# pearl-robot-lab/2HandedAfforder

Measured on AMD Instinct MI355X. Metric: affordance frames/sec/GPU @1024^2, 32-tok prompt; mask IoU vs ref, higher is better.
Workload: dtype bf16

## Files before the change

2handedafforder_amd/csrc/window_attention.hip:

```cpp
#include "haff_common.h"

#ifndef HAFF_TUNING
#undef HAFF_WIN_NOKREAD
#undef HAFF_WIN_NOVREAD
#undef HAFF_WIN_NOSCR
#undef HAFF_WIN_NODMA
#undef HAFF_WIN_RS
#undef HAFF_WIN_KLAST_OLD
#endif

namespace {

struct WinArgs {
  const bf16_t *q, *k, *v;
  bf16_t* o;
  long q_sb, q_sh, q_st;
  long k_sb, k_sh, k_st;
  long v_sb, v_sh, v_st;
  long o_sb, o_sh, o_st;
  int B, H;
  float scale;
  const bf16_t *tab_h, *tab_w;
  int grid_h, grid_w, wps;
  long pad_token;
};

#ifdef HAFF_WIN_TRACE
__device__ unsigned long long haff_win_trace_buf[64 * 16];
#define WTRACE(i) do { if (blockIdx.x == 0 && tid == 0 && it < 64) haff_win_trace_buf[it * 16 + (i)] = wall_clock64(); } while (0)
#else
#define WTRACE(i) do {} while (0)
#endif

constexpr float WLOG2E = 1.4426950408889634f;
typedef __attribute__((address_space(3))) bf16x4* wlds_v4_ptr;
typedef const __attribute__((address_space(1))) void* wgptr_t;
typedef __attribute__((address_space(3))) void* wlptr_t;
__device__ __attribute__((aligned(16))) unsigned int haff_win_zero_page[4];

template <int D, int S>
struct WinCfg {
  static constexpr int N = S * S;
  static constexpr int NKD = (D + 31) / 32;
  static constexpr int ND = D / 16;
  static constexpr int CPR = D / 8;
  static constexpr int KPC = (D * 2) % 64 == 32 ? 0 : 2;
  static constexpr int KSTR = D * 2 + 16 * KPC;
  static constexpr int VSTR = D * 2;
  static constexpr int NKS = (S + 1) / 2;
#ifdef HAFF_WIN_RS
  static constexpr int RS = HAFF_WIN_RS;
#else
  static constexpr int RS = 52;
#endif
  static constexpr int QPW = 2;
  static constexpr int NWAVES = (S + QPW - 1) / QPW;
  static constexpr int NTHREADS = 64 * NWAVES;
  static constexpr int KSLOTS = N * (CPR + KPC), VSLOTS = N * CPR;
  static constexpr int K_BYTES = N * KSTR, V_BYTES = N * VSTR;
  static constexpr int PAD_SLOTS = (KSLOTS + VSLOTS + 63) / 64 * 64;
  static constexpr int BUF_BYTES = PAD_SLOTS * 16;
  static constexpr int SC_BYTES = NWAVES * 16 * RS * 4;
  static constexpr int LDS_BYTES = 2 * BUF_BYTES + SC_BYTES;
};

template <int D, int S, bool F16 = false>
__global__ __launch_bounds__((WinCfg<D, S>::NTHREADS)) void window_attn_kernel(WinArgs p) {
  using E = h16<F16>;
  using C = WinCfg<D, S>;
  static_assert(D % 16 == 0 && D <= 96 && S <= 16 && 2 * S - 1 <= 32, "window kernel geometry");
  extern __shared__ __attribute__((aligned(16))) unsigned char wsm[];
  float* sScr = reinterpret_cast<float*>(wsm + 2 * C::BUF_BYTES);

  const int tid = threadIdx.x;
  const int lane = tid & 63;
  const int wave = __builtin_amdgcn_readfirstlane(tid >> 6);
  const int fr = lane & 15, fh = lane >> 4;
  const int n_items = p.B * p.H;

  auto decode = [&](int id, int& win, int& h) {
    if ((p.B & 7) == 0) {
      const int x = id & 7, kseq = id >> 3;
      win = (kseq / p.H) * 8 + x;
      h = kseq - (kseq / p.H) * p.H;
    } else {
      win = id / p.H;
      h = id - win * p.H;
    }
  };

  constexpr int TOTAL_SLOTS = C::KSLOTS + C::VSLOTS;
  constexpr int NDMA = (C::PAD_SLOTS + C::NTHREADS - 1) / C::NTHREADS;
  static_assert((C::K_BYTES % 16) == 0 && C::KSTR == (C::CPR + C::KPC) * 16 && C::VSTR == C::CPR * 16 && C::KSTR % 64 == 32, "slot layout");
  unsigned slot_off[NDMA];
  unsigned slot_pad[NDMA];
  const long v_minus_k = (p.v - p.k);
  const unsigned vmk_bytes = (unsigned)(v_minus_k * 2);
#pragma unroll
  for (int i = 0; i < NDMA; ++i) {
    const int sl = tid + i * C::NTHREADS;
    long off;
    unsigned pad = 0;
    if (sl >= TOTAL_SLOTS) {
      off = 0;
    } else if (sl < C::KSLOTS) {
      const int row = sl / (C::CPR + C::KPC), c = sl - row * (C::CPR + C::KPC);
      off = (long)row * p.k_st + (c < C::CPR ? c * 8 : 0);
      pad = ((unsigned)(row / S) << 28) | ((unsigned)(row % S) << 24) | (unsigned)((c < C::CPR ? c : 0) * 16);
    } else {
      const int sv = sl - C::KSLOTS;
      const int row = sv / C::CPR, c = sv - row * C::CPR;
      off = v_minus_k + (long)row * p.v_st + c * 8;
      pad = ((unsigned)(row / S) << 28) | ((unsigned)(row % S) << 24) | (1u << 23) | (unsigned)(c * 16);
    }
    slot_off[i] = (unsigned)(off * 2);
    slot_pad[i] = pad;
  }
  uint4 qnext[C::QPW][C::NKD];
  const int qcol = min(fr, S - 1);
  const bf16_t* nx_kb = p.k;
  int nx_pad_h0 = S, nx_pad_w0 = S;
  unsigned nx_pad_base = 0, nx_lds0 = 0;
  auto begin_loads = [&](int id, int buf) {
    int win, h;
    decode(id, win, h);
    const bf16_t* qb = p.q + (long)win * p.q_sb + (long)h * p.q_sh;
    const bf16_t* kb = p.k + (long)win * p.k_sb + (long)h * p.k_sh;
    int pad_h0 = S, pad_w0 = S;
    if (p.grid_h > 0) {
      const int wi = win % (p.wps * p.wps);
      pad_h0 = p.grid_h - (wi / p.wps) * S;
      pad_w0 = p.grid_w - (wi % p.wps) * S;
    }
    const unsigned pad_base = (unsigned)((p.pad_token * p.k_st - (long)win * p.k_sb) * 2);
    const bf16_t* qpad = p.q + p.pad_token * p.q_st + (long)h * p.q_sh;
#pragma unroll
    for (int t = 0; t < C::QPW; ++t) {
      const int qh_t = min(wave + t * C::NWAVES, S - 1);
      const bf16_t* qsrc = (qh_t >= pad_h0 || qcol >= pad_w0) ? qpad : qb + (long)(qh_t * S + qcol) * p.q_st;
#pragma unroll
      for (int kd = 0; kd < C::NKD; ++kd) {
        const int col = kd * 32 + fh * 8;
        qnext[t][kd] = make_uint4(0, 0, 0, 0);
        if (col < D) qnext[t][kd] = *reinterpret_cast<const uint4*>(qsrc + col);
      }
    }
    nx_kb = kb;
    nx_pad_h0 = pad_h0;
    nx_pad_w0 = pad_w0;
    nx_pad_base = pad_base;
    nx_lds0 = (unsigned)(uintptr_t)(wlptr_t)(wsm + buf * C::BUF_BYTES) + wave * 1024;
  };
  auto issue_dma = [&](int i0, int i1) {
#pragma unroll
    for (int i = 0; i < NDMA; ++i) {
      if (i < i0 || i >= i1) continue;
      const unsigned m0v = nx_lds0 + i * C::NTHREADS * 16;
      const bool is_pad = (int)(slot_pad[i] >> 28) >= nx_pad_h0 || (int)((slot_pad[i] >> 24) & 15u) >= nx_pad_w0;
      const unsigned off = is_pad ? nx_pad_base + (slot_pad[i] & 0xffu) + ((slot_pad[i] >> 23) & 1u) * vmk_bytes : slot_off[i];
#ifdef HAFF_WIN_NODMA
      asm volatile("" ::"v"(off), "s"(m0v));
      continue;
#endif
      if ((i + 1) * C::NTHREADS <= C::PAD_SLOTS || (i * C::NTHREADS + wave * 64) < C::PAD_SLOTS)
        asm volatile("s_mov_b32 m0, %2\n\ts_nop 0\n\tglobal_load_lds_dwordx4 %0, %1" ::"v"(off), "s"(nx_kb), "s"(m0v)
                     : "memory");
    }
  };
  constexpr int DMA_Q1 = (NDMA + 3) / 4, DMA_Q2 = (NDMA + 1) / 2, DMA_Q3 = (3 * NDMA + 3) / 4;

  auto settle_q = [&]() {
#pragma unroll
    for (int t = 0; t < C::QPW; ++t)
#pragma unroll
      for (int kd = 0; kd < C::NKD; ++kd)
        asm volatile("" : "+v"(qnext[t][kd].x), "+v"(qnext[t][kd].y), "+v"(qnext[t][kd].z), "+v"(qnext[t][kd].w));
  };

  int item = blockIdx.x;
  if (item >= n_items) return;
  begin_loads(item, 0);
  issue_dma(0, NDMA);

  bf16x8 th[2][C::NKD], tw[2][C::NKD];
#pragma unroll
  for (int mt = 0; mt < 2; ++mt) {
    const int r = min(mt * 16 + fr, 2 * S - 2);
#pragma unroll
    for (int kd = 0; kd < C::NKD; ++kd) {
      const int col = kd * 32 + fh * 8;
      uint4 a = make_uint4(0, 0, 0, 0), b = make_uint4(0, 0, 0, 0);
      if (col < D) {
        a = *reinterpret_cast<const uint4*>(p.tab_h + r * D + col);
        b = *reinterpret_cast<const uint4*>(p.tab_w + r * D + col);
      }
      th[mt][kd] = __builtin_bit_cast(bf16x8, a);
      tw[mt][kd] = __builtin_bit_cast(bf16x8, b);
    }
  }
  asm volatile("s_waitcnt vmcnt(0)" ::: "memory");
  settle_q();
#pragma unroll
  for (int mt = 0; mt < 2; ++mt)
#pragma unroll
    for (int kd = 0; kd < C::NKD; ++kd) {
      asm volatile("" : "+v"(th[mt][kd]));
      asm volatile("" : "+v"(tw[mt][kd]));
    }
  __syncthreads();

  const float sl2 = p.scale * WLOG2E;
  float* scr = sScr + wave * (16 * C::RS);
  const int tr_q = fr >> 2, tr_p = fr & 3;
  bool kw_ok[4];
#pragma unroll
  for (int j = 0; j < 4; ++j) kw_ok[j] = (4 * fh + j) < S;

  for (int it = 0;; ++it) {
    const int buf = it & 1;
    const unsigned char* sK = wsm + buf * C::BUF_BYTES;
    const unsigned char* sV = sK + C::K_BYTES;
    int win, h;
    decode(item, win, h);
    bf16_t* ob = p.o + (long)win * p.o_sb + (long)h * p.o_sh;
    uint4 qcur[C::QPW][C::NKD];
#pragma unroll
    for (int t = 0; t < C::QPW; ++t)
#pragma unroll
      for (int kd = 0; kd < C::NKD; ++kd) qcur[t][kd] = qnext[t][kd];
    const int next = item + gridDim.x;
    const bool has_next = next < n_items;
    WTRACE(0);
    if (has_next) {
      begin_loads(next, buf ^ 1);
      issue_dma(0, DMA_Q1);
    }
    WTRACE(1);

#pragma unroll
    for (int t = 0; t < C::QPW; ++t) {
      const int qh = wave + t * C::NWAVES;
      static_assert(C::QPW * C::NWAVES == S, "q-tiles must divide evenly over the waves");
      bf16x8 qraw[C::NKD], qs[C::NKD];
#pragma unroll
      for (int kd = 0; kd < C::NKD; ++kd) {
        const uint4 r = qcur[t][kd];
        uint4 rs = make_uint4(0, 0, 0, 0);
        if (kd * 32 + fh * 8 < D) {
          float qv[8];
          const unsigned w4[4] = {r.x, r.y, r.z, r.w};
#pragma unroll
          for (int j = 0; j < 4; ++j) {
            qv[2 * j] = E::lo(w4[j]) * sl2;
            qv[2 * j + 1] = E::hi(w4[j]) * sl2;
          }
          rs.x = E::pack2(qv[0], qv[1]); rs.y = E::pack2(qv[2], qv[3]);
          rs.z = E::pack2(qv[4], qv[5]); rs.w = E::pack2(qv[6], qv[7]);
        }
        qraw[kd] = __builtin_bit_cast(bf16x8, r);
        qs[kd] = __builtin_bit_cast(bf16x8, rs);
      }

      float relw4[4], relh_t[S];
      {
        f32x4 t0 = f32x4{0.f, 0.f, 0.f, 0.f}, t1 = t0;
#pragma unroll
        for (int kd = 0; kd < C::NKD; ++kd) {
          t0 = E::mfma16(tw[0][kd], qraw[kd], t0);
          t1 = E::mfma16(tw[1][kd], qraw[kd], t1);
        }
        float a[4] = {t0[0], t0[1], t0[2], t0[3]}, b[4] = {t1[0], t1[1], t1[2], t1[3]};
#ifdef HAFF_WIN_NOSCR
#pragma unroll
        for (int j = 0; j < 4; ++j) relw4[j] = kw_ok[j] ? (a[j] + b[j]) * WLOG2E : -INFINITY;
#else
        store4(scr + fr * C::RS + 4 * fh, a);
        store4(scr + fr * C::RS + 16 + 4 * fh, b);
        __builtin_amdgcn_wave_barrier();
#pragma unroll
        for (int j = 0; j < 4; ++j) {
          const int r = min(max(qcol - (4 * fh + j) + S - 1, 0), 2 * S - 2);
          relw4[j] = kw_ok[j] ? scr[fr * C::RS + r] * WLOG2E : -INFINITY;
        }
        __builtin_amdgcn_wave_barrier();
#endif
      }
      {
        f32x4 t0 = f32x4{0.f, 0.f, 0.f, 0.f}, t1 = t0;
#pragma unroll
        for (int kd = 0; kd < C::NKD; ++kd) {
          t0 = E::mfma16(th[0][kd], qraw[kd], t0);
          t1 = E::mfma16(th[1][kd], qraw[kd], t1);
        }
        float a[4] = {t0[0], t0[1], t0[2], t0[3]}, b[4] = {t1[0], t1[1], t1[2], t1[3]};
#ifdef HAFF_WIN_NOSCR
#pragma unroll
        for (int kt = 0; kt < S; ++kt) relh_t[kt] = (a[kt & 3] + b[kt & 3]) * WLOG2E;
#else
        store4(scr + fr * C::RS + 4 * fh, a);
        store4(scr + fr * C::RS + 16 + 4 * fh, b);
        __builtin_amdgcn_wave_barrier();
#pragma unroll
        for (int kt = 0; kt < S; ++kt) relh_t[kt] = scr[fr * C::RS + (qh - kt + S - 1)] * WLOG2E;
        __builtin_amdgcn_wave_barrier();
#endif
      }

      WTRACE(2 + 5 * t);
      f32x4 sacc[S];
#pragma unroll
      for (int kt = 0; kt < S; ++kt)
        sacc[kt] = f32x4{relw4[0] + relh_t[kt], relw4[1] + relh_t[kt], relw4[2] + relh_t[kt], relw4[3] + relh_t[kt]};
      constexpr int KG = (S + 1) / 2;
#ifdef HAFF_WIN_KLAST_OLD
      const int koff_last = min(fh * 16 + (C::NKD - 1) * 64, D * 2 - 16);
#else
      const int koff_last = (D * 2 - (C::NKD - 1) * 64 == 32) ? (C::NKD - 1) * 64 - 32 + ((fh + 2) & 3) * 16
                                                              : min(fh * 16 + (C::NKD - 1) * 64, D * 2 - 16);
#endif
#pragma unroll
      for (int g0 = 0; g0 < S; g0 += KG) {
#pragma unroll
        for (int kd = 0; kd < C::NKD; ++kd) {
#pragma unroll
          for (int kt = g0; kt < g0 + KG && kt < S; ++kt) {
#ifdef HAFF_WIN_NOKREAD
            const bf16x8 kf = qs[(kd + 1) % C::NKD];
#else
            const bf16x8 kf = *reinterpret_cast<const bf16x8*>(sK + (kt * S + qcol) * C::KSTR + (kd == C::NKD - 1 ? koff_last : fh * 16 + kd * 64));
#endif
            sacc[kt] = E::mfma16(kf, qs[kd], sacc[kt]);
          }
        }
        __builtin_amdgcn_sched_barrier(0);
      }

      WTRACE(3 + 5 * t);
      if (has_next) {
        if (t == 0) issue_dma(DMA_Q1, DMA_Q2);
        else issue_dma(DMA_Q3, NDMA);
      }
      float mx = -1e30f;
#pragma unroll
      for (int kt = 0; kt < S; ++kt)
#pragma unroll
        for (int j = 0; j < 4; ++j) mx = fmaxf(mx, sacc[kt][j]);
      mx = fmaxf(mx, __shfl_xor(mx, 16, 64));
      mx = fmaxf(mx, __shfl_xor(mx, 32, 64));
      float psum = 0.f;
#pragma unroll
      for (int kt = 0; kt < S; ++kt)
#pragma unroll
        for (int j = 0; j < 4; ++j) {
          const float e = __builtin_amdgcn_exp2f(sacc[kt][j] - mx);
          sacc[kt][j] = e;
          psum += e;
        }
      psum += __shfl_xor(psum, 16, 64);
      psum += __shfl_xor(psum, 32, 64);

      WTRACE(4 + 5 * t);
      f32x4 oacc[C::ND];
#pragma unroll
      for (int dt = 0; dt < C::ND; ++dt) oacc[dt] = f32x4{0.f, 0.f, 0.f, 0.f};
      const int vkw = min(4 * fh + tr_q, S - 1);
#pragma unroll
      for (int ks = 0; ks < C::NKS; ++ks) {
        constexpr int dummy = 0; (void)dummy;
        const int t0 = 2 * ks, t1 = (2 * ks + 1 < S) ? 2 * ks + 1 : 2 * ks;
        uint4 u;
        u.x = E::pack2(sacc[t0][0], sacc[t0][1]);
        u.y = E::pack2(sacc[t0][2], sacc[t0][3]);
        u.z = (2 * ks + 1 < S) ? E::pack2(sacc[t1][0], sacc[t1][1]) : 0u;
        u.w = (2 * ks + 1 < S) ? E::pack2(sacc[t1][2], sacc[t1][3]) : 0u;
        const bf16x8 pf = __builtin_bit_cast(bf16x8, u);
        const unsigned char* v0 = sV + (t0 * S + vkw) * C::VSTR + 8 * tr_p;
        const unsigned char* v1 = sV + (t1 * S + vkw) * C::VSTR + 8 * tr_p;
#pragma unroll
        for (int dt = 0; dt < C::ND; ++dt) {
#ifdef HAFF_WIN_NOVREAD
          const bf16x8 vf = qs[dt % C::NKD];
          asm volatile("" ::"v"(v0), "v"(v1));
#else
          const bf16x4 lo = __builtin_amdgcn_ds_read_tr16_b64_v4i16((wlds_v4_ptr)(v0 + 32 * dt));
          const bf16x4 hi = __builtin_amdgcn_ds_read_tr16_b64_v4i16((wlds_v4_ptr)(v1 + 32 * dt));
          const bf16x8 vf = __builtin_shufflevector(lo, hi, 0, 1, 2, 3, 4, 5, 6, 7);
#endif
          oacc[dt] = E::mfma16(vf, pf, oacc[dt]);
        }
      }

      WTRACE(5 + 5 * t);
      if (has_next && t == 0) issue_dma(DMA_Q2, DMA_Q3);
      const float inv = 1.0f / psum;
      if (fr < S) {
        bf16_t* orow = ob + (long)(qh * S + fr) * p.o_st + 4 * fh;
#pragma unroll
        for (int dt = 0; dt < C::ND; ++dt) {
          float v[4] = {oacc[dt][0] * inv, oacc[dt][1] * inv, oacc[dt][2] * inv, oacc[dt][3] * inv};
          store4h<F16>(orow + 16 * dt, v);
        }
      }
    }

    WTRACE(12);
    if (!has_next) break;
    item = next;
    asm volatile("s_waitcnt vmcnt(0)" ::: "memory");
    settle_q();
    WTRACE(13);
    __syncthreads();
    WTRACE(14);
  }
}

}

#ifdef HAFF_WIN_TRACE
extern "C" int haff_win_trace_read(unsigned long long* host, int n_words) {
  return hipMemcpyFromSymbol(host, HIP_SYMBOL(haff_win_trace_buf), sizeof(unsigned long long) * n_words) == hipSuccess ? 0 : 1;
}
#endif

template <bool F16 = false>
static int window_attention_impl(const void* q, long q_sb, long q_sh, long q_st,
                                 const void* k, long k_sb, long k_sh, long k_st,
                                 const void* v, long v_sb, long v_sh, long v_st,
                                 void* o, long o_sb, long o_sh, long o_st,
                                 int n_windows, int H, int S, int d, float scale,
                                 const void* tab_h, const void* tab_w, int grid_h, int grid_w,
                                 long pad_token, void* stream) {
  if (n_windows <= 0 || H <= 0 || S <= 0 || d <= 0 || !tab_h || !tab_w) return HAFF_ERR_BAD_ARG;
  if ((q_st & 7) || (k_st & 7) || (v_st & 7) || (o_st & 3) || (q_sh & 7) || (k_sh & 7) || (v_sh & 7) || (o_sh & 3) ||
      (q_sb & 7) || (k_sb & 7) || (v_sb & 7) || (o_sb & 3))
    return HAFF_ERR_BAD_ARG;
  if ((reinterpret_cast<uintptr_t>(q) & 15) || (reinterpret_cast<uintptr_t>(k) & 15) ||
      (reinterpret_cast<uintptr_t>(v) & 15) || (reinterpret_cast<uintptr_t>(o) & 7) ||
      (reinterpret_cast<uintptr_t>(tab_h) & 15) || (reinterpret_cast<uintptr_t>(tab_w) & 15))
    return HAFF_ERR_BAD_ARG;
  if (S != 14 || d != 80) return HAFF_ERR_UNSUPPORTED;
  if (k_sb != v_sb || k_sh != v_sh || k_st != v_st) return HAFF_ERR_UNSUPPORTED;
  {
    const long dvk = reinterpret_cast<const bf16_t*>(v) - reinterpret_cast<const bf16_t*>(k);
    const long span = (dvk < 0 ? -dvk : dvk) + (long)S * S * k_st + d;
    if (dvk < 0 || span * 2 >= (1L << 32)) return HAFF_ERR_UNSUPPORTED;
  }
  WinArgs p{reinterpret_cast<const bf16_t*>(q), reinterpret_cast<const bf16_t*>(k), reinterpret_cast<const bf16_t*>(v),
            reinterpret_cast<bf16_t*>(o), q_sb, q_sh, q_st, k_sb, k_sh, k_st, v_sb, v_sh, v_st, o_sb, o_sh, o_st,
            n_windows, H, scale, reinterpret_cast<const bf16_t*>(tab_h), reinterpret_cast<const bf16_t*>(tab_w),
            grid_h, grid_w, grid_h > 0 ? (grid_h + S - 1) / S : 0, pad_token};
  if (grid_h > 0) {
    if (grid_w != grid_h || (n_windows % (p.wps * p.wps)) != 0 || pad_token < 0 || q_st != k_st ||
        (pad_token + 1) * k_st * 2 >= (1L << 32) || pad_token * k_st < (long)(n_windows - 1) * k_sb)
      return HAFF_ERR_BAD_ARG;
    const long dvk = reinterpret_cast<const bf16_t*>(v) - reinterpret_cast<const bf16_t*>(k);
    if ((pad_token * k_st + dvk + d) * 2 >= (1L << 32)) return HAFF_ERR_UNSUPPORTED;
  }
  using C = WinCfg<80, 14>;
  if (hipFuncSetAttribute(reinterpret_cast<const void*>(&window_attn_kernel<80, 14, F16>),
                          hipFuncAttributeMaxDynamicSharedMemorySize, C::LDS_BYTES) != hipSuccess)
    return HAFF_ERR_LAUNCH;
  const int n_items = n_windows * H;
  dim3 grid(n_items < 256 ? n_items : 256), block(C::NTHREADS);
  hipLaunchKernelGGL((window_attn_kernel<80, 14, F16>), grid, block, C::LDS_BYTES, reinterpret_cast<hipStream_t>(stream), p);
  return haff_check_launch();
}

extern "C" int haff_window_attention_bf16(const void* q, long q_sb, long q_sh, long q_st,
                                          const void* k, long k_sb, long k_sh, long k_st,
                                          const void* v, long v_sb, long v_sh, long v_st,
                                          void* o, long o_sb, long o_sh, long o_st,
                                          int n_windows, int H, int S, int d, float scale,
                                          const void* tab_h, const void* tab_w, int grid_h, int grid_w,
                                          long pad_token, void* stream) {
  return window_attention_impl(q, q_sb, q_sh, q_st, k, k_sb, k_sh, k_st, v, v_sb, v_sh, v_st, o, o_sb, o_sh, o_st, n_windows, H, S,
                               d, scale, tab_h, tab_w, grid_h, grid_w, pad_token, stream);
}

extern "C" int haff_window_attention_f16(const void* q, long q_sb, long q_sh, long q_st,
                                         const void* k, long k_sb, long k_sh, long k_st,
                                         const void* v, long v_sb, long v_sh, long v_st,
                                         void* o, long o_sb, long o_sh, long o_st,
                                         int n_windows, int H, int S, int d, float scale,
                                         const void* tab_h, const void* tab_w, int grid_h, int grid_w,
                                         long pad_token, void* stream) {
  return window_attention_impl<true>(q, q_sb, q_sh, q_st, k, k_sb, k_sh, k_st, v, v_sb, v_sh, v_st, o, o_sb, o_sh, o_st, n_windows, H,
                                     S, d, scale, tab_h, tab_w, grid_h, grid_w, pad_token, stream);
// ... 2 lines not shown
```

2handedafforder_amd/lib.py:

```python
import ctypes
import os
import subprocess

_HERE = os.path.dirname(os.path.abspath(__file__))
LIB_PATH = os.environ.get("HAFF_LIB_PATH") or os.path.join(_HERE, "lib", "libhaff_hip.so")
CSRC_DIR = os.path.join(_HERE, "csrc")

c_void_p, c_long, c_int, c_float = ctypes.c_void_p, ctypes.c_long, ctypes.c_int, ctypes.c_float

_PROTOS = {
    "haff_gemm_bf16": [c_void_p, c_long, c_void_p, c_long, c_void_p, c_long, c_void_p, c_void_p, c_long, c_void_p,
                       c_int, c_int, c_int, c_int, c_int, c_int, c_void_p],
    "haff_gemm_bf16_cfg": [c_void_p, c_long, c_void_p, c_long, c_void_p, c_long, c_void_p, c_void_p, c_long, c_void_p,
                           c_int, c_int, c_int, c_int, c_int, c_int, c_int, c_void_p],
    "haff_gemm_bf16_ws": [c_void_p, c_long, c_void_p, c_long, c_void_p, c_long, c_void_p, c_void_p, c_long, c_void_p,
                          c_int, c_int, c_int, c_int, c_int, c_int, c_void_p, c_long, c_void_p],
    "haff_gemm_bf16_rms": [c_void_p, c_long, c_void_p, c_long, c_void_p, c_long, c_void_p, c_void_p, c_long, c_int, c_int, c_int,
                           c_int, c_int, c_int, c_void_p, c_int, c_float, c_void_p, c_void_p, c_void_p],
    "haff_gemm_bf16_gather": [c_void_p, c_long, c_void_p, c_long, c_void_p, c_long, c_void_p, c_long, c_void_p, c_void_p,
                              c_long, c_void_p, c_int, c_int, c_int, c_int, c_int, c_int, c_void_p],
    "haff_gemm_bf16_ln": [c_void_p, c_long, c_void_p, c_long, c_void_p, c_long, c_void_p, c_void_p, c_long, c_void_p,
                          c_void_p, c_void_p, c_int, c_int, c_int, c_int, c_int, c_int, c_void_p],
    "haff_gemm_bf16_heads": [c_void_p, c_long, c_void_p, c_long, c_void_p, c_void_p, c_void_p, c_void_p, c_void_p, c_int, c_int, c_int,
                             c_int, c_int, c_long, c_long, c_void_p],
# ... 43 lines not shown
                           c_void_p, c_long, c_long, c_long, c_void_p, c_long, c_long, c_long,
                           c_int, c_int, c_int, c_int, c_int, c_float, c_int, c_int, c_void_p, c_void_p, c_int,
                           c_void_p],
    "haff_attention_decode_rows_bf16": [c_void_p, c_long, c_long, c_void_p, c_long, c_long, c_long, c_void_p, c_long, c_long, c_long,
                                        c_void_p, c_long, c_long, c_int, c_int, c_int, c_int, c_float, c_void_p, c_void_p],
    "haff_attention_decode_rows_f16": [c_void_p, c_long, c_long, c_void_p, c_long, c_long, c_long, c_void_p, c_long, c_long, c_long,
                                       c_void_p, c_long, c_long, c_int, c_int, c_int, c_int, c_float, c_void_p, c_void_p],
    "haff_attention_decode_rows_f32": [c_void_p, c_long, c_long, c_void_p, c_long, c_long, c_long, c_void_p, c_long, c_long, c_long,
                                       c_void_p, c_long, c_long, c_int, c_int, c_int, c_int, c_float, c_void_p, c_void_p],
    "haff_decode_attention_rope_rows_bf16": [c_void_p, c_long, c_void_p, c_void_p, c_void_p, c_void_p, c_int, c_int, c_int, c_int,
                                             c_float, c_void_p, c_void_p],
    "haff_decode_attention_rope_rows_f16": [c_void_p, c_long, c_void_p, c_void_p, c_void_p, c_void_p, c_int, c_int, c_int, c_int,
                                            c_float, c_void_p, c_void_p],
    "haff_rope_cache_rows": [c_void_p, c_long, c_void_p, c_void_p, c_void_p, c_int, c_int, c_int, c_int, c_int, c_void_p,
                             c_int, c_int, c_void_p],
    "haff_relpos_tables": [c_void_p, c_long, c_long, c_long, c_void_p, c_void_p, c_void_p, c_void_p,
                           c_int, c_int, c_int, c_int, c_int, c_void_p],
    "haff_relpos_tables_bf16": [c_void_p, c_long, c_long, c_long, c_void_p, c_void_p, c_void_p, c_void_p,
                                c_int, c_int, c_int, c_int, c_void_p],
    "haff_window_attention_bf16": [c_void_p, c_long, c_long, c_long, c_void_p, c_long, c_long, c_long,
                                   c_void_p, c_long, c_long, c_long, c_void_p, c_long, c_long, c_long,
                                   c_int, c_int, c_int, c_int, c_float, c_void_p, c_void_p, c_int, c_int, c_long,
                                   c_void_p],
    "haff_window_attention_f16": [c_void_p, c_long, c_long, c_long, c_void_p, c_long, c_long, c_long,
                                   c_void_p, c_long, c_long, c_long, c_void_p, c_long, c_long, c_long,
                                   c_int, c_int, c_int, c_int, c_float, c_void_p, c_void_p, c_int, c_int, c_long,
                                   c_void_p],
    "haff_attention_lse_bf16": [c_void_p, c_long, c_long, c_long, c_void_p, c_long, c_long, c_long, c_void_p, c_long, c_long, c_long,
                                c_void_p, c_long, c_long, c_long, c_int, c_int, c_int, c_int, c_int, c_float, c_int, c_int,
                                c_void_p, c_void_p],
    "haff_attention_bwd_bf16": [c_void_p, c_void_p, c_void_p, c_void_p, c_void_p, c_void_p, c_void_p, c_void_p, c_void_p,
                                c_void_p, c_long, c_long, c_int, c_int, c_int, c_int, c_int, c_float, c_int, c_int, c_void_p],
    "haff_gemm_tn_workspace_elems": [c_long, c_int, c_int],
    "haff_gemm_tn_bf16": [c_void_p, c_long, c_void_p, c_long, c_long, c_int, c_int, c_void_p, c_long, c_void_p, c_int, c_void_p],
    "haff_lora_qkv_rope_fwd": [c_void_p, c_long, c_void_p, c_long, c_void_p, c_void_p, c_int, c_void_p, c_void_p, c_void_p, c_void_p,
                               c_long, c_long, c_int, c_int, c_int, c_float, c_void_p],
    "haff_lora_qkv_rope_bwd": [c_void_p, c_void_p, c_void_p, c_long, c_void_p, c_void_p, c_long, c_long, c_int, c_int, c_int, c_void_p],
    "haff_lora_dx": [c_void_p, c_long, c_void_p, c_long, c_void_p, c_long, c_void_p, c_long, c_int, c_long, c_int, c_float, c_void_p],
    "haff_lora_dx2": [c_void_p, c_long, c_void_p, c_long, c_void_p, c_void_p, c_long, c_void_p, c_long, c_int, c_long, c_int, c_float,
                      c_void_p],
    "haff_lora_tn_workspace_elems": [c_long, c_int, c_int],
    "haff_lora_tn": [c_void_p, c_long, c_int, c_void_p, c_long, c_long, c_int, c_void_p, c_long, c_void_p, c_long, c_int, c_int,
                     c_int, c_float, c_void_p],
    "haff_global_attention_bf16": [c_void_p, c_long, c_long, c_long, c_void_p, c_long, c_long, c_long,
                                   c_void_p, c_long, c_long, c_long, c_void_p, c_long, c_long, c_long,
                                   c_int, c_int, c_int, c_int, c_float, c_void_p, c_void_p, c_void_p],
# ... 121 lines not shown
```

include/haff_hip.h:

```cpp
#ifndef HAFF_HIP_H
#define HAFF_HIP_H

#ifdef __cplusplus
extern "C" {
#endif

int haff_gemm_bf16(const void* A, long lda, const void* W, long ldw, void* C, long ldc, const float* bias,
                   const void* resid, long ldr, const int* row_map, int M, int N, int K, int act, int out_f32,
                   int swiglu, void* stream);
int haff_gemm_bf16_cfg(const void* A, long lda, const void* W, long ldw, void* C, long ldc, const float* bias,
                       const void* resid, long ldr, const int* row_map, int M, int N, int K, int act, int out_f32,
                       int swiglu, int tile_cfg, void* stream);
int haff_gemm_bf16_ws(const void* A, long lda, const void* W, long ldw, void* C, long ldc, const float* bias,
                      const void* resid, long ldr, const int* row_map, int M, int N, int K, int act, int out_f32,
                      int swiglu, void* workspace, long workspace_bytes, void* stream);
int haff_gemm_f16(const void* A, long lda, const void* W, long ldw, void* C, long ldc, const float* bias,
                  const void* resid, long ldr, const int* row_map, int M, int N, int K, int act, int out_f32,
                  int swiglu, void* stream);
int haff_gemm_f16_cfg(const void* A, long lda, const void* W, long ldw, void* C, long ldc, const float* bias,
                      const void* resid, long ldr, const int* row_map, int M, int N, int K, int act, int out_f32,
                      int swiglu, int tile_cfg, void* stream);
int haff_gemm_f16_ws(const void* A, long lda, const void* W, long ldw, void* C, long ldc, const float* bias,
                     const void* resid, long ldr, const int* row_map, int M, int N, int K, int act, int out_f32,
                     int swiglu, void* workspace, long workspace_bytes, void* stream);
// ... 89 lines not shown

int haff_gemm_tn_workspace_elems(long M, int N1, int N2);
int haff_gemm_tn_bf16(const void* A, long lda, const void* B, long ldb, long M, int N1, int N2, float* workspace,
                      long workspace_elems, void* out, int out_f32, void* stream);

int haff_lora_qkv_rope_fwd(const void* qkv, long ld_qkv, const void* tT, long ldt, const void* Bq, const void* Bv, int ldb,
                           const float* cos_sin, void* q_out, void* k_out, void* v_out, long ldo, long M, int H, int d, int T,
                           float scale, void* stream);
int haff_lora_qkv_rope_bwd(const void* dq, const void* dk, const void* dv, long ld_in, const float* cos_sin, void* dqkv,
                           long ld_out, long M, int H, int d, int T, void* stream);
int haff_lora_dx(const void* dtT, long ldt, const void* A2, long lda, const void* keep, long ldk, void* dx, long ldx,
                 int accumulate, long M, int K, float scale, void* stream);
int haff_lora_dx2(const void* dtT, long ldt, const void* A2, long lda, const void* keep_q, const void* keep_v, long ldk, void* dx,
                  long ldx, int accumulate, long M, int K, float scale, void* stream);
int haff_lora_tn_workspace_elems(long M, int R, int N);
int haff_lora_tn(const void* sT, long lds, int R, const void* big, long ldb, long M, int N, float* workspace,
                 long workspace_elems, void* out, long ldo, int out_f32, int transposed, int j_valid, float scale, void* stream);

int haff_window_attention_bf16(const void* q, long q_sb, long q_sh, long q_st, const void* k, long k_sb, long k_sh,
                               long k_st, const void* v, long v_sb, long v_sh, long v_st, void* o, long o_sb,
                               long o_sh, long o_st, int n_windows, int H, int S, int d, float scale,
                               const void* tab_h, const void* tab_w, int grid_h, int grid_w, long pad_token,
                               void* stream);
int haff_window_attention_f16(const void* q, long q_sb, long q_sh, long q_st, const void* k, long k_sb, long k_sh,
                              long k_st, const void* v, long v_sb, long v_sh, long v_st, void* o, long o_sb,
                              long o_sh, long o_st, int n_windows, int H, int S, int d, float scale,
                              const void* tab_h, const void* tab_w, int grid_h, int grid_w, long pad_token,
                              void* stream);

int haff_global_attention_bf16(const void* q, long q_sb, long q_sh, long q_st, const void* k, long k_sb, long k_sh,
                               long k_st, const void* v, long v_sb, long v_sh, long v_st, void* o, long o_sb,
                               long o_sh, long o_st, int B, int H, int S, int d, float scale,
                               const void* tab_h, const void* tab_w, void* stream);
int haff_global_attention_f16(const void* q, long q_sb, long q_sh, long q_st, const void* k, long k_sb, long k_sh,
                              long k_st, const void* v, long v_sb, long v_sh, long v_st, void* o, long o_sb,
                              long o_sh, long o_st, int B, int H, int S, int d, float scale,
                              const void* tab_h, const void* tab_w, void* stream);

int haff_layernorm(const void* x, long ldx, void* y, long ldy, const float* w, const float* b, const int* in_map,
                   int rows, int C, float eps, int dtype, void* stream);
int haff_rmsnorm(const void* x, long ldx, void* y, long ldy, const float* w, int rows, int C, float eps, int dtype,
                 void* stream);
int haff_row_stats(const void* x, long ldx, float* stats, int rows, int C, float eps, int rms, int dtype, void* stream);

int haff_row_stats_finalize(const float* partials, float* stats, int rows, int slots, int C, float eps, void* stream);

// ... 91 lines not shown
```

Measured before the change: 112.3.

## Rework window attention to 32x32 MFMA tiles over 8 waves with LDS rel-pos tables

Result: no change. 112.4 (median of 6 runs) (+0.1%).

```diff
diff --git a/2handedafforder_amd/csrc/window_attention.hip b/2handedafforder_amd/csrc/window_attention.hip
--- a/2handedafforder_amd/csrc/window_attention.hip
+++ b/2handedafforder_amd/csrc/window_attention.hip
@@ -1,13 +1,4 @@
 #include "haff_common.h"
-
-#ifndef HAFF_TUNING
-#undef HAFF_WIN_NOKREAD
-#undef HAFF_WIN_NOVREAD
-#undef HAFF_WIN_NOSCR
-#undef HAFF_WIN_NODMA
-#undef HAFF_WIN_RS
-#undef HAFF_WIN_KLAST_OLD
-#endif
 
 namespace {
 
@@ -34,64 +25,59 @@
 
 constexpr float WLOG2E = 1.4426950408889634f;
 typedef __attribute__((address_space(3))) bf16x4* wlds_v4_ptr;
-typedef const __attribute__((address_space(1))) void* wgptr_t;
 typedef __attribute__((address_space(3))) void* wlptr_t;
-__device__ __attribute__((aligned(16))) unsigned int haff_win_zero_page[4];
 
 template <int D, int S>
 struct WinCfg {
   static constexpr int N = S * S;
-  static constexpr int NKD = (D + 31) / 32;
-  static constexpr int ND = D / 16;
+  static constexpr int NKS = D / 16;
+  static constexpr int NDT = (D + 31) / 32;
+  static constexpr int NKT = S / 2;
+  static constexpr int NT = 2 * S - 1;
   static constexpr int CPR = D / 8;
-  static constexpr int KPC = (D * 2) % 64 == 32 ? 0 : 2;
-  static constexpr int KSTR = D * 2 + 16 * KPC;
-  static constexpr int VSTR = D * 2;
-  static constexpr int NKS = (S + 1) / 2;
-#ifdef HAFF_WIN_RS
-  static constexpr int RS = HAFF_WIN_RS;
-#else
-  static constexpr int RS = 52;
-#endif
-  static constexpr int QPW = 2;
-  static constexpr int NWAVES = (S + QPW - 1) / QPW;
+  static constexpr int RSTR = D * 2;
+  static constexpr int NWAVES = 8;
   static constexpr int NTHREADS = 64 * NWAVES;
-  static constexpr int KSLOTS = N * (CPR + KPC), VSLOTS = N * CPR;
-  static constexpr int K_BYTES = N * KSTR, V_BYTES = N * VSTR;
+  static constexpr int KSLOTS = N * CPR, VSLOTS = N * CPR;
+  static constexpr int K_BYTES = N * RSTR;
   static constexpr int PAD_SLOTS = (KSLOTS + VSLOTS + 63) / 64 * 64;
   static constexpr int BUF_BYTES = PAD_SLOTS * 16;
-  static constexpr int SC_BYTES = NWAVES * 16 * RS * 4;
-  static constexpr int LDS_BYTES = 2 * BUF_BYTES + SC_BYTES;
+  static constexpr int TAB_BYTES = 2 * NT * RSTR;
+  static constexpr int RS = NT;
+  static constexpr int SC_BYTES = NWAVES * 32 * RS * 4;
+  static constexpr int LDS_BYTES = 2 * BUF_BYTES + TAB_BYTES + SC_BYTES;
+  static_assert(D % 16 == 0 && D <= 96 && S % 2 == 0 && S <= 16 && NT <= 32, "window kernel geometry");
+  static_assert(LDS_BYTES <= 160 * 1024, "LDS");
+  static_assert(2 * K_BYTES + (16 - S) * RSTR + 64 * NDT <= BUF_BYTES, "masked-key reads stay inside the buffer");
 };
 
 template <int D, int S, bool F16 = false>
 __global__ __launch_bounds__((WinCfg<D, S>::NTHREADS)) void window_attn_kernel(WinArgs p) {
   using E = h16<F16>;
   using C = WinCfg<D, S>;
-  static_assert(D % 16 == 0 && D <= 96 && S <= 16 && 2 * S - 1 <= 32, "window kernel geometry");
   extern __shared__ __attribute__((aligned(16))) unsigned char wsm[];
-  float* sScr = reinterpret_cast<float*>(wsm + 2 * C::BUF_BYTES);
+  unsigned char* sTab = wsm + 2 * C::BUF_BYTES;
+  float* sScr = reinterpret_cast<float*>(sTab + C::TAB_BYTES);
 
   const int tid = threadIdx.x;
   const int lane = tid & 63;
   const int wave = __builtin_amdgcn_readfirstlane(tid >> 6);
-  const int fr = lane & 15, fh = lane >> 4;
+  const int c32 = lane & 31, h = lane >> 5;
   const int n_items = p.B * p.H;
 
-  auto decode = [&](int id, int& win, int& h) {
+  auto decode = [&](int id, int& win, int& hd) {
     if ((p.B & 7) == 0) {
       const int x = id & 7, kseq = id >> 3;
       win = (kseq / p.H) * 8 + x;
-      h = kseq - (kseq / p.H) * p.H;
+      hd = kseq - (kseq / p.H) * p.H;
     } else {
       win = id / p.H;
-      h = id - win * p.H;
+      hd = id - win * p.H;
     }
   };
 
   constexpr int TOTAL_SLOTS = C::KSLOTS + C::VSLOTS;
   constexpr int NDMA = (C::PAD_SLOTS + C::NTHREADS - 1) / C::NTHREADS;
-  static_assert((C::K_BYTES % 16) == 0 && C::KSTR == (C::CPR + C::KPC) * 16 && C::VSTR == C::CPR * 16 && C::KSTR % 64 == 32, "slot layout");
   unsigned slot_off[NDMA];
   unsigned slot_pad[NDMA];
   const long v_minus_k = (p.v - p.k);
@@ -104,9 +90,9 @@
     if (sl >= TOTAL_SLOTS) {
       off = 0;
     } else if (sl < C::KSLOTS) {
-      const int row = sl / (C::CPR + C::KPC), c = sl - row * (C::CPR + C::KPC);
-      off = (long)row * p.k_st + (c < C::CPR ? c * 8 : 0);
-      pad = ((unsigned)(row / S) << 28) | ((unsigned)(row % S) << 24) | (unsigned)((c < C::CPR ? c : 0) * 16);
+      const int row = sl / C::CPR, c = (sl - row * C::CPR) ^ ((row / S) & 1);
+      off = (long)row * p.k_st + c * 8;
+      pad = ((unsigned)(row / S) << 28) | ((unsigned)(row % S) << 24) | (unsigned)(c * 16);
     } else {
       const int sv = sl - C::KSLOTS;
       const int row = sv / C::CPR, c = sv - row * C::CPR;
@@ -116,16 +102,19 @@
     slot_off[i] = (unsigned)(off * 2);
     slot_pad[i] = pad;
   }
-  uint4 qnext[C::QPW][C::NKD];
-  const int qcol = min(fr, S - 1);
+
+  const int q0 = wave * C::N / C::NWAVES, qn = (wave + 1) * C::N / C::NWAVES - q0;
+  const int qidx = q0 + min(c32, qn - 1);
+  const int qh = qidx / S, qw = qidx - (qidx / S) * S;
+  uint4 qnext[C::NKS];
   const bf16_t* nx_kb = p.k;
   int nx_pad_h0 = S, nx_pad_w0 = S;
   unsigned nx_pad_base = 0, nx_lds0 = 0;
   auto begin_loads = [&](int id, int buf) {
-    int win, h;
-    decode(id, win, h);
-    const bf16_t* qb = p.q + (long)win * p.q_sb + (long)h * p.q_sh;
-    const bf16_t* kb = p.k + (long)win * p.k_sb + (long)h * p.k_sh;
+    int win, hd;
+    decode(id, win, hd);
+    const bf16_t* qb = p.q + (long)win * p.q_sb + (long)hd * p.q_sh;
+    const bf16_t* kb = p.k + (long)win * p.k_sb + (long)hd * p.k_sh;
     int pad_h0 = S, pad_w0 = S;
     if (p.grid_h > 0) {
       const int wi = win % (p.wps * p.wps);
@@ -133,18 +122,10 @@
       pad_w0 = p.grid_w - (wi % p.wps) * S;
     }
     const unsigned pad_base = (unsigned)((p.pad_token * p.k_st - (long)win * p.k_sb) * 2);
-    const bf16_t* qpad = p.q + p.pad_token * p.q_st + (long)h * p.q_sh;
-#pragma unroll
-    for (int t = 0; t < C::QPW; ++t) {
-      const int qh_t = min(wave + t * C::NWAVES, S - 1);
-      const bf16_t* qsrc = (qh_t >= pad_h0 || qcol >= pad_w0) ? qpad : qb + (long)(qh_t * S + qcol) * p.q_st;
-#pragma unroll
-      for (int kd = 0; kd < C::NKD; ++kd) {
-        const int col = kd * 32 + fh * 8;
-        qnext[t][kd] = make_uint4(0, 0, 0, 0);
-        if (col < D) qnext[t][kd] = *reinterpret_cast<const uint4*>(qsrc + col);
-      }
-    }
+    const bf16_t* qpad = p.q + p.pad_token * p.q_st + (long)hd * p.q_sh;
+    const bf16_t* qsrc = (qh >= pad_h0 || qw >= pad_w0) ? qpad : qb + (long)qidx * p.q_st;
+#pragma unroll
+    for (int ks = 0; ks < C::NKS; ++ks) qnext[ks] = *reinterpret_cast<const uint4*>(qsrc + ks * 16 + h * 8);
     nx_kb = kb;
     nx_pad_h0 = pad_h0;
     nx_pad_w0 = pad_w0;
@@ -158,23 +139,17 @@
       const unsigned m0v = nx_lds0 + i * C::NTHREADS * 16;
       const bool is_pad = (int)(slot_pad[i] >> 28) >= nx_pad_h0 || (int)((slot_pad[i] >> 24) & 15u) >= nx_pad_w0;
       const unsigned off = is_pad ? nx_pad_base + (slot_pad[i] & 0xffu) + ((slot_pad[i] >> 23) & 1u) * vmk_bytes : slot_off[i];
-#ifdef HAFF_WIN_NODMA
-      asm volatile("" ::"v"(off), "s"(m0v));
-      continue;
-#endif
       if ((i + 1) * C::NTHREADS <= C::PAD_SLOTS || (i * C::NTHREADS + wave * 64) < C::PAD_SLOTS)
         asm volatile("s_mov_b32 m0, %2\n\ts_nop 0\n\tglobal_load_lds_dwordx4 %0, %1" ::"v"(off), "s"(nx_kb), "s"(m0v)
                      : "memory");
     }
   };
-  constexpr int DMA_Q1 = (NDMA + 3) / 4, DMA_Q2 = (NDMA + 1) / 2, DMA_Q3 = (3 * NDMA + 3) / 4;
+  constexpr int DMA_Q0 = NDMA / 2, DMA_Q1 = 3 * NDMA / 4;
 
   auto settle_q = [&]() {
 #pragma unroll
-    for (int t = 0; t < C::QPW; ++t)
-#pragma unroll
-      for (int kd = 0; kd < C::NKD; ++kd)
-        asm volatile("" : "+v"(qnext[t][kd].x), "+v"(qnext[t][kd].y), "+v"(qnext[t][kd].z), "+v"(qnext[t][kd].w));
+    for (int ks = 0; ks < C::NKS; ++ks)
+      asm volatile("" : "+v"(qnext[ks].x), "+v"(qnext[ks].y), "+v"(qnext[ks].z), "+v"(qnext[ks].w));
   };
 
   int item = blockIdx.x;
@@ -182,231 +157,175 @@
   begin_loads(item, 0);
   issue_dma(0, NDMA);
 
-  bf16x8 th[2][C::NKD], tw[2][C::NKD];
-#pragma unroll
-  for (int mt = 0; mt < 2; ++mt) {
-    const int r = min(mt * 16 + fr, 2 * S - 2);
-#pragma unroll
-    for (int kd = 0; kd < C::NKD; ++kd) {
-      const int col = kd * 32 + fh * 8;
-      uint4 a = make_uint4(0, 0, 0, 0), b = make_uint4(0, 0, 0, 0);
-      if (col < D) {
-        a = *reinterpret_cast<const uint4*>(p.tab_h + r * D + col);
-        b = *reinterpret_cast<const uint4*>(p.tab_w + r * D + col);
-      }
-      th[mt][kd] = __builtin_bit_cast(bf16x8, a);
-      tw[mt][kd] = __builtin_bit_cast(bf16x8, b);
-    }
+  for (int i = tid; i < 2 * C::NT * C::CPR; i += C::NTHREADS) {
+    const int t = i / (C::NT * C::CPR), rc = i - t * (C::NT * C::CPR);
+    const uint4 x = *reinterpret_cast<const uint4*>((t ? p.tab_w : p.tab_h) + rc * 8);
+    *reinterpret_cast<uint4*>(sTab + i * 16) = x;
   }
   asm volatile("s_waitcnt vmcnt(0)" ::: "memory");
   settle_q();
-#pragma unroll
-  for (int mt = 0; mt < 2; ++mt)
-#pragma unroll
-    for (int kd = 0; kd < C::NKD; ++kd) {
-      asm volatile("" : "+v"(th[mt][kd]));
-      asm volatile("" : "+v"(tw[mt][kd]));
-    }
   __syncthreads();
 
   const float sl2 = p.scale * WLOG2E;
-  float* scr = sScr + wave * (16 * C::RS);
-  const int tr_q = fr >> 2, tr_p = fr & 3;
-  bool kw_ok[4];
-#pragma unroll
-  for (int j = 0; j < 4; ++j) kw_ok[j] = (4 * fh + j) < S;
+  float* scr = sScr + wave * (32 * C::RS);
+  const int kw_a = 2 * (c32 & 3) + ((c32 >> 2) & 1) + 8 * ((c32 >> 3) & 1);
+  const int k_row_a = (c32 >> 4) * S + kw_a;
+  const int k_chunk_sw = (c32 >> 4) & 1;
+  const int tr_g = (lane >> 4) & 1, tr_q = (lane >> 2) & 3, tr_p = lane & 3;
+  const int v_lane = (2 * tr_q + h) * C::RSTR + (16 * tr_g + 4 * tr_p) * 2;
+  auto kw_dead = [](int i) { return 2 * ((i & 7) & 3) + 8 * ((i & 7) >> 2) >= S; };
+  bool kw_ok[8];
+#pragma unroll
+  for (int m = 0; m < 8; ++m) kw_ok[m] = (2 * (m & 3) + h + 8 * (m >> 2)) < S;
 
   for (int it = 0;; ++it) {
     const int buf = it & 1;
     const unsigned char* sK = wsm + buf * C::BUF_BYTES;
     const unsigned char* sV = sK + C::K_BYTES;
-    int win, h;
-    decode(item, win, h);
-    bf16_t* ob = p.o + (long)win * p.o_sb + (long)h * p.o_sh;
-    uint4 qcur[C::QPW][C::NKD];
-#pragma unroll
-    for (int t = 0; t < C::QPW; ++t)
-#pragma unroll
-      for (int kd = 0; kd < C::NKD; ++kd) qcur[t][kd] = qnext[t][kd];
+    int win, hd;
+    decode(item, win, hd);
+    bf16_t* ob = p.o + (long)win * p.o_sb + (long)hd * p.o_sh;
+    bf16x8 qraw[C::NKS];
+#pragma unroll
+    for (int ks = 0; ks < C::NKS; ++ks) qraw[ks] = __builtin_bit_cast(bf16x8, qnext[ks]);
     const int next = item + gridDim.x;
     const bool has_next = next < n_items;
     WTRACE(0);
     if (has_next) {
       begin_loads(next, buf ^ 1);
-      issue_dma(0, DMA_Q1);
+      issue_dma(0, DMA_Q0);
     }
     WTRACE(1);
 
-#pragma unroll
-    for (int t = 0; t < C::QPW; ++t) {
-      const int qh = wave + t * C::NWAVES;
-      static_assert(C::QPW * C::NWAVES == S, "q-tiles must divide evenly over the waves");
-      bf16x8 qraw[C::NKD], qs[C::NKD];
-#pragma unroll
-      for (int kd = 0; kd < C::NKD; ++kd) {
-        const uint4 r = qcur[t][kd];
-        uint4 rs = make_uint4(0, 0, 0, 0);
-        if (kd * 32 + fh * 8 < D) {
-          float qv[8];
-          const unsigned w4[4] = {r.x, r.y, r.z, r.w};
-#pragma unroll
-          for (int j = 0; j < 4; ++j) {
-            qv[2 * j] = E::lo(w4[j]) * sl2;
-            qv[2 * j + 1] = E::hi(w4[j]) * sl2;
-          }
-          rs.x = E::pack2(qv[0], qv[1]); rs.y = E::pack2(qv[2], qv[3]);
-          rs.z = E::pack2(qv[4], qv[5]); rs.w = E::pack2(qv[6], qv[7]);
+    float relw[8], relh[S];
+    {
+      f32x16 tw = {}, th = {};
+#pragma unroll
+      for (int ks = 0; ks < C::NKS; ++ks) {
+        const int row = min(c32, C::NT - 1);
+        const bf16x8 ah = *reinterpret_cast<const bf16x8*>(sTab + row * C::RSTR + (2 * ks + h) * 16);
+        const bf16x8 aw = *reinterpret_cast<const bf16x8*>(sTab + (C::NT + row) * C::RSTR + (2 * ks + h) * 16);
+        th = E::mfma32(ah, qraw[ks], th);
+        tw = E::mfma32(aw, qraw[ks], tw);
+      }
+#pragma unroll
+      for (int i = 0; i < 16; ++i) {
+        const int r = (i & 3) + 8 * (i >> 2) + 4 * h;
+        if (r < C::NT) scr[c32 * C::RS + r] = tw[i];
+      }
+      __builtin_amdgcn_wave_barrier();
+#pragma unroll
+      for (int m = 0; m < 8; ++m) {
+        const int kw = 2 * (m & 3) + h + 8 * (m >> 2);
+        relw[m] = kw_ok[m] ? scr[c32 * C::RS + min(max(qw - kw + S - 1, 0), C::NT - 1)] * WLOG2E : -INFINITY;
+      }
+      __builtin_amdgcn_wave_barrier();
+#pragma unroll
+      for (int i = 0; i < 16; ++i) {
+        const int r = (i & 3) + 8 * (i >> 2) + 4 * h;
+        if (r < C::NT) scr[c32 * C::RS + r] = th[i];
+      }
+      __builtin_amdgcn_wave_barrier();
+#pragma unroll
+      for (int kh = 0; kh < S; ++kh) relh[kh] = scr[c32 * C::RS + qh - kh + S - 1] * WLOG2E;
+      __builtin_amdgcn_wave_barrier();
+    }
+    if (has_next) issue_dma(DMA_Q0, DMA_Q1);
+    bf16x8 qs[C::NKS];
+#pragma unroll
+    for (int ks = 0; ks < C::NKS; ++ks) {
+      const uint4 r = __builtin_bit_cast(uint4, qraw[ks]);
+      const unsigned w4[4] = {r.x, r.y, r.z, r.w};
+      uint4 rs;
+      rs.x = E::pack2(E::lo(w4[0]) * sl2, E::hi(w4[0]) * sl2);
+      rs.y = E::pack2(E::lo(w4[1]) * sl2, E::hi(w4[1]) * sl2);
+      rs.z = E::pack2(E::lo(w4[2]) * sl2, E::hi(w4[2]) * sl2);
+      rs.w = E::pack2(E::lo(w4[3]) * sl2, E::hi(w4[3]) * sl2);
+      qs[ks] = __builtin_bit_cast(bf16x8, rs);
+    }
+
+    WTRACE(2);
+    f32x16 sacc[C::NKT];
+#pragma unroll
+    for (int kt = 0; kt < C::NKT; ++kt)
+#pragma unroll
+      for (int i = 0; i < 16; ++i) sacc[kt][i] = relw[i & 7] + relh[2 * kt + (i >> 3)];
+#pragma unroll
+    for (int kt = 0; kt < C::NKT; ++kt) {
+      const unsigned char* krow = sK + (2 * kt * S + k_row_a) * C::RSTR;
+#pragma unroll
+      for (int ks = 0; ks < C::NKS; ++ks) {
+        const bf16x8 kf = *reinterpret_cast<const bf16x8*>(krow + ((2 * ks + h) ^ k_chunk_sw) * 16);
+        sacc[kt] = E::mfma32(kf, qs[ks], sacc[kt]);
+      }
+    }
+
+    WTRACE(3);
+    if (has_next) issue_dma(DMA_Q1, NDMA);
+    float mx = -1e30f;
+#pragma unroll
+    for (int kt = 0; kt < C::NKT; ++kt)
+#pragma unroll
+      for (int i = 0; i < 16; ++i)
+        if (!kw_dead(i)) mx = fmaxf(mx, sacc[kt][i]);
+    mx = fmaxf(mx, __shfl_xor(mx, 32, 64));
+    float psum = 0.f;
+    uint4 pk[C::NKT][2];
+#pragma unroll
+    for (int kt = 0; kt < C::NKT; ++kt) {
+      float e[16];
+#pragma unroll
+      for (int i = 0; i < 16; ++i) {
+        e[i] = kw_dead(i) ? 0.f : __builtin_amdgcn_exp2f(sacc[kt][i] - mx);
+        psum += e[i];
+      }
+#pragma unroll
+      for (int s = 0; s < 2; ++s) {
+        pk[kt][s].x = E::pack2(e[8 * s + 0], e[8 * s + 1]);
+        pk[kt][s].y = E::pack2(e[8 * s + 2], e[8 * s + 3]);
+        pk[kt][s].z = E::pack2(e[8 * s + 4], e[8 * s + 5]);
+        pk[kt][s].w = E::pack2(e[8 * s + 6], e[8 * s + 7]);
+      }
+    }
+    psum += __shfl_xor(psum, 32, 64);
+
+    WTRACE(4);
+    f32x16 oacc[C::NDT];
+#pragma unroll
+    for (int dt = 0; dt < C::NDT; ++dt) oacc[dt] = f32x16{};
+#pragma unroll
+    for (int kt = 0; kt < C::NKT; ++kt)
+#pragma unroll
+      for (int s = 0; s < 2; ++s) {
+        const bf16x8 pf = __builtin_bit_cast(bf16x8, pk[kt][s]);
+        const unsigned char* vb = sV + (2 * kt + s) * S * C::RSTR + v_lane;
+#pragma unroll
+        for (int dt = 0; dt < C::NDT; ++dt) {
+          const bf16x4 lo = __builtin_amdgcn_ds_read_tr16_b64_v4i16((wlds_v4_ptr)(vb + 64 * dt));
+          const bf16x4 hi = __builtin_amdgcn_ds_read_tr16_b64_v4i16((wlds_v4_ptr)(vb + 8 * C::RSTR + 64 * dt));
+          const bf16x8 vf = __builtin_shufflevector(lo, hi, 0, 1, 2, 3, 4, 5, 6, 7);
+          oacc[dt] = E::mfma32(vf, pf, oacc[dt]);
         }
-        qraw[kd] = __builtin_bit_cast(bf16x8, r);
-        qs[kd] = __builtin_bit_cast(bf16x8, rs);
-      }
-
-      float relw4[4], relh_t[S];
-      {
-        f32x4 t0 = f32x4{0.f, 0.f, 0.f, 0.f}, t1 = t0;
-#pragma unroll
-        for (int kd = 0; kd < C::NKD; ++kd) {
-          t0 = E::mfma16(tw[0][kd], qraw[kd], t0);
-          t1 = E::mfma16(tw[1][kd], qraw[kd], t1);
+      }
+
+    WTRACE(5);
+    const float inv = 1.0f / psum;
+    if (c32 < qn) {
+      bf16_t* orow = ob + (long)(q0 + c32) * p.o_st + 4 * h;
+#pragma unroll
+      for (int dt = 0; dt < C::NDT; ++dt)
+#pragma unroll
+        for (int g = 0; g < 4; ++g) {
+          if (32 * dt + 8 * g >= D) continue;
+          float v[4] = {oacc[dt][4 * g] * inv, oacc[dt][4 * g + 1] * inv, oacc[dt][4 * g + 2] * inv, oacc[dt][4 * g + 3] * inv};
+          store4h<F16>(orow + 32 * dt + 8 * g, v);
         }
-        float a[4] = {t0[0], t0[1], t0[2], t0[3]}, b[4] = {t1[0], t1[1], t1[2], t1[3]};
-#ifdef HAFF_WIN_NOSCR
-#pragma unroll
-        for (int j = 0; j < 4; ++j) relw4[j] = kw_ok[j] ? (a[j] + b[j]) * WLOG2E : -INFINITY;
-#else
-        store4(scr + fr * C::RS + 4 * fh, a);
-        store4(scr + fr * C::RS + 16 + 4 * fh, b);
-        __builtin_amdgcn_wave_barrier();
-#pragma unroll
-        for (int j = 0; j < 4; ++j) {
-          const int r = min(max(qcol - (4 * fh + j) + S - 1, 0), 2 * S - 2);
-          relw4[j] = kw_ok[j] ? scr[fr * C::RS + r] * WLOG2E : -INFINITY;
-        }
-        __builtin_amdgcn_wave_barrier();
-#endif
-      }
-      {
-        f32x4 t0 = f32x4{0.f, 0.f, 0.f, 0.f}, t1 = t0;
-#pragma unroll
-        for (int kd = 0; kd < C::NKD; ++kd) {
-          t0 = E::mfma16(th[0][kd], qraw[kd], t0);
-          t1 = E::mfma16(th[1][kd], qraw[kd], t1);
-        }
-        float a[4] = {t0[0], t0[1], t0[2], t0[3]}, b[4] = {t1[0], t1[1], t1[2], t1[3]};
-#ifdef HAFF_WIN_NOSCR
-#pragma unroll
-        for (int kt = 0; kt < S; ++kt) relh_t[kt] = (a[kt & 3] + b[kt & 3]) * WLOG2E;
-#else
-        store4(scr + fr * C::RS + 4 * fh, a);
-        store4(scr + fr * C::RS + 16 + 4 * fh, b);
-        __builtin_amdgcn_wave_barrier();
-#pragma unroll
-        for (int kt = 0; kt < S; ++kt) relh_t[kt] = scr[fr * C::RS + (qh - kt + S - 1)] * WLOG2E;
-        __builtin_amdgcn_wave_barrier();
-#endif
-      }
-
-      WTRACE(2 + 5 * t);
-      f32x4 sacc[S];
-#pragma unroll
-      for (int kt = 0; kt < S; ++kt)
-        sacc[kt] = f32x4{relw4[0] + relh_t[kt], relw4[1] + relh_t[kt], relw4[2] + relh_t[kt], relw4[3] + relh_t[kt]};
-      constexpr int KG = (S + 1) / 2;
-#ifdef HAFF_WIN_KLAST_OLD
-      const int koff_last = min(fh * 16 + (C::NKD - 1) * 64, D * 2 - 16);
-#else
-      const int koff_last = (D * 2 - (C::NKD - 1) * 64 == 32) ? (C::NKD - 1) * 64 - 32 + ((fh + 2) & 3) * 16
-                                                              : min(fh * 16 + (C::NKD - 1) * 64, D * 2 - 16);
-#endif
-#pragma unroll
-      for (int g0 = 0; g0 < S; g0 += KG) {
-#pragma unroll
-        for (int kd = 0; kd < C::NKD; ++kd) {
-#pragma unroll
-          for (int kt = g0; kt < g0 + KG && kt < S; ++kt) {
-#ifdef HAFF_WIN_NOKREAD
-            const bf16x8 kf = qs[(kd + 1) % C::NKD];
-#else
-            const bf16x8 kf = *reinterpret_cast<const bf16x8*>(sK + (kt * S + qcol) * C::KSTR + (kd == C::NKD - 1 ? koff_last : fh * 16 + kd * 64));
-#endif
-            sacc[kt] = E::mfma16(kf, qs[kd], sacc[kt]);
-          }
-        }
-        __builtin_amdgcn_sched_barrier(0);
-      }
-
-      WTRACE(3 + 5 * t);
-      if (has_next) {
-        if (t == 0) issue_dma(DMA_Q1, DMA_Q2);
-        else issue_dma(DMA_Q3, NDMA);
-      }
-      float mx = -1e30f;
-#pragma unroll
-      for (int kt = 0; kt < S; ++kt)
-#pragma unroll
-        for (int j = 0; j < 4; ++j) mx = fmaxf(mx, sacc[kt][j]);
-      mx = fmaxf(mx, __shfl_xor(mx, 16, 64));
-      mx = fmaxf(mx, __shfl_xor(mx, 32, 64));
-      float psum = 0.f;
-#pragma unroll
-      for (int kt = 0; kt < S; ++kt)
-#pragma unroll
-        for (int j = 0; j < 4; ++j) {
-          const float e = __builtin_amdgcn_exp2f(sacc[kt][j] - mx);
-          sacc[kt][j] = e;
-          psum += e;
-        }
-      psum += __shfl_xor(psum, 16, 64);
-      psum += __shfl_xor(psum, 32, 64);
-
-      WTRACE(4 + 5 * t);
-      f32x4 oacc[C::ND];
-#pragma unroll
-      for (int dt = 0; dt < C::ND; ++dt) oacc[dt] = f32x4{0.f, 0.f, 0.f, 0.f};
-      const int vkw = min(4 * fh + tr_q, S - 1);
-#pragma unroll
-      for (int ks = 0; ks < C::NKS; ++ks) {
-        constexpr int dummy = 0; (void)dummy;
-        const int t0 = 2 * ks, t1 = (2 * ks + 1 < S) ? 2 * ks + 1 : 2 * ks;
-        uint4 u;
-        u.x = E::pack2(sacc[t0][0], sacc[t0][1]);
-        u.y = E::pack2(sacc[t0][2], sacc[t0][3]);
-        u.z = (2 * ks + 1 < S) ? E::pack2(sacc[t1][0], sacc[t1][1]) : 0u;
-        u.w = (2 * ks + 1 < S) ? E::pack2(sacc[t1][2], sacc[t1][3]) : 0u;
-        const bf16x8 pf = __builtin_bit_cast(bf16x8, u);
-        const unsigned char* v0 = sV + (t0 * S + vkw) * C::VSTR + 8 * tr_p;
-        const unsigned char* v1 = sV + (t1 * S + vkw) * C::VSTR + 8 * tr_p;
-#pragma unroll
-        for (int dt = 0; dt < C::ND; ++dt) {
-#ifdef HAFF_WIN_NOVREAD
-          const bf16x8 vf = qs[dt % C::NKD];
-          asm volatile("" ::"v"(v0), "v"(v1));
-#else
-          const bf16x4 lo = __builtin_amdgcn_ds_read_tr16_b64_v4i16((wlds_v4_ptr)(v0 + 32 * dt));
-          const bf16x4 hi = __builtin_amdgcn_ds_read_tr16_b64_v4i16((wlds_v4_ptr)(v1 + 32 * dt));
-          const bf16x8 vf = __builtin_shufflevector(lo, hi, 0, 1, 2, 3, 4, 5, 6, 7);
-#endif
-          oacc[dt] = E::mfma16(vf, pf, oacc[dt]);
-        }
-      }
-
-      WTRACE(5 + 5 * t);
-      if (has_next && t == 0) issue_dma(DMA_Q2, DMA_Q3);
-      const float inv = 1.0f / psum;
-      if (fr < S) {
-        bf16_t* orow = ob + (long)(qh * S + fr) * p.o_st + 4 * fh;
-#pragma unroll
-        for (int dt = 0; dt < C::ND; ++dt) {
-          float v[4] = {oacc[dt][0] * inv, oacc[dt][1] * inv, oacc[dt][2] * inv, oacc[dt][3] * inv};
-          store4h<F16>(orow + 16 * dt, v);
-        }
-      }
-    }
-
-    WTRACE(12);
+    }
+
+    WTRACE(6);
     if (!has_next) break;
     item = next;
-    asm volatile("s_waitcnt vmcnt(0)" ::: "memory");
+    asm volatile("s_waitcnt vmcnt(0) lgkmcnt(0)" ::: "memory");
     settle_q();
     WTRACE(13);
     __syncthreads();
@@ -421,6 +340,17 @@
   return hipMemcpyFromSymbol(host, HIP_SYMBOL(haff_win_trace_buf), sizeof(unsigned long long) * n_words) == hipSuccess ? 0 : 1;
 }
 #endif
+
+extern "C" int haff_window_attention_geometry(int n_windows, int H, int S, int d, int* out3) {
+  if (!out3 || n_windows <= 0 || H <= 0) return HAFF_ERR_BAD_ARG;
+  if (S != 14 || d != 80) return HAFF_ERR_UNSUPPORTED;
+  using C = WinCfg<80, 14>;
+  const long n_items = (long)n_windows * H;
+  out3[0] = (int)(n_items < 256 ? n_items : 256);
+  out3[1] = C::NTHREADS;
+  out3[2] = C::LDS_BYTES;
+  return 0;
+}
 
 template <bool F16 = false>
 static int window_attention_impl(const void* q, long q_sb, long q_sh, long q_st,
@@ -460,9 +390,9 @@
   if (hipFuncSetAttribute(reinterpret_cast<const void*>(&window_attn_kernel<80, 14, F16>),
                           hipFuncAttributeMaxDynamicSharedMemorySize, C::LDS_BYTES) != hipSuccess)
     return HAFF_ERR_LAUNCH;
-  const int n_items = n_windows * H;
-  dim3 grid(n_items < 256 ? n_items : 256), block(C::NTHREADS);
-  hipLaunchKernelGGL((window_attn_kernel<80, 14, F16>), grid, block, C::LDS_BYTES, reinterpret_cast<hipStream_t>(stream), p);
+  int geo[3];
+  haff_window_attention_geometry(n_windows, H, S, d, geo);
+  hipLaunchKernelGGL((window_attn_kernel<80, 14, F16>), dim3(geo[0]), dim3(geo[1]), geo[2], reinterpret_cast<hipStream_t>(stream), p);
   return haff_check_launch();
 }
 
diff --git a/2handedafforder_amd/lib.py b/2handedafforder_amd/lib.py
--- a/2handedafforder_amd/lib.py
+++ b/2handedafforder_amd/lib.py
@@ -89,6 +89,7 @@
                                    c_void_p, c_long, c_long, c_long, c_void_p, c_long, c_long, c_long,
                                    c_int, c_int, c_int, c_int, c_float, c_void_p, c_void_p, c_int, c_int, c_long,
                                    c_void_p],
+    "haff_window_attention_geometry": [c_int, c_int, c_int, c_int, c_void_p],
     "haff_window_attention_f16": [c_void_p, c_long, c_long, c_long, c_void_p, c_long, c_long, c_long,
                                    c_void_p, c_long, c_long, c_long, c_void_p, c_long, c_long, c_long,
                                    c_int, c_int, c_int, c_int, c_float, c_void_p, c_void_p, c_int, c_int, c_long,
diff --git a/include/haff_hip.h b/include/haff_hip.h
--- a/include/haff_hip.h
+++ b/include/haff_hip.h
@@ -135,6 +135,7 @@
                                long o_sh, long o_st, int n_windows, int H, int S, int d, float scale,
                                const void* tab_h, const void* tab_w, int grid_h, int grid_w, long pad_token,
                                void* stream);
+int haff_window_attention_geometry(int n_windows, int H, int S, int d, int* out3);
 int haff_window_attention_f16(const void* q, long q_sb, long q_sh, long q_st, const void* k, long k_sb, long k_sh,
                               long k_st, const void* v, long v_sb, long v_sh, long v_st, void* o, long o_sb,
                               long o_sh, long o_st, int n_windows, int H, int S, int d, float scale,
```
